# latentnetworks/vimure

Hardware: AMD Instinct MI355X
Metric: CAVI iterations/sec (L=4 N=2000 M=200 K=2 synthetic, mutuality on) (higher is better)
Workload: dtype f64

## Files before the change

### vimure_amd/build.py

```python
import os
import subprocess
from concurrent.futures import ThreadPoolExecutor

HERE = os.path.dirname(os.path.abspath(__file__))
ROOT = os.path.dirname(HERE)
CSRC = os.path.join(HERE, "csrc")
OBJ = os.path.join(CSRC, "_obj")
LIB = os.environ.get("VMR_LIB_OUT", os.path.join(HERE, "libvimure_hip.so"))
HIPCC = os.environ.get("HIPCC", "/opt/rocm/bin/hipcc")
HOST_SRC = os.path.join(CSRC, "host_init.c")
HOST_LIB = os.path.join(HERE, "libvimure_host.so")
HEADERS = [os.path.join(CSRC, "vmr_internal.h"), os.path.join(CSRC, "sweep_sl.h"), os.path.join(CSRC, "sweep_gen.h"),
           os.path.join(CSRC, "sample_draw.h"), os.path.join(CSRC, "report_draw.h"), os.path.join(CSRC, "ppc_layer.h"), os.path.join(CSRC, "rho_row.h"),
           os.path.join(CSRC, "report_lik.h"), os.path.join(CSRC, "read_side.h"), os.path.join(CSRC, "sampled_side.h"),
           os.path.join(ROOT, "include", "vimure_hip.h")]
KS = (2, 3, 4, 5, 6, 7, 8)
FLAGS = ["-O3", "--offload-arch=gfx950", "-fPIC", "-std=c++17", "-I" + os.path.join(ROOT, "include"), "-I" + CSRC]


def units(dev=False):
    extra = ["-DVMR_DEV"] if dev else []
    u = [("vimure_hip", os.path.join(CSRC, "vimure_hip.hip"), extra),
         ("sorted_lists", os.path.join(CSRC, "sorted_lists.hip"), extra),
         ("sweep_gen", os.path.join(CSRC, "sweep_gen.hip"), extra),
         ("generate", os.path.join(CSRC, "generate.hip"), extra),
         ("draw_prior", os.path.join(CSRC, "draw_prior.hip"), extra),
         ("ppc", os.path.join(CSRC, "ppc.hip"), extra),
         ("netstats", os.path.join(CSRC, "netstats.hip"), extra),
         ("triads", os.path.join(CSRC, "triads.hip"), extra),
         ("mixing", os.path.join(CSRC, "mixing.hip"), extra),
         ("ppc_rep", os.path.join(CSRC, "ppc_rep.hip"), extra),
         ("edge_table", os.path.join(CSRC, "edge_table.hip"), extra),
         ("score_truth", os.path.join(CSRC, "score_truth.hip"), extra),
         ("reporter_table", os.path.join(CSRC, "reporter_table.hip"), extra),
         ("heldout", os.path.join(CSRC, "heldout.hip"), extra),
         ("report_scores", os.path.join(CSRC, "report_scores.hip"), extra),
         ("influence", os.path.join(CSRC, "influence.hip"), extra)]
    dev_ks = tuple(int(k) for k in os.environ.get("VMR_DEV_KS", "2").split(","))
    for k in (dev_ks if dev else KS):
        u.append((f"sweep_sl_k{k}", os.path.join(CSRC, "sweep_sl.hip"), extra + [f"-DVMR_K={k}"]))
    return u


def _stale(obj, src):
    if not os.path.exists(obj):
        return True
    t = os.path.getmtime(obj)
    return any(os.path.getmtime(d) > t for d in [src] + HEADERS)


def needs_build() -> bool:
    dev = bool(os.environ.get("VMR_DEV"))
    tag = os.path.join(OBJ, "dev" if dev else "full")
    if not os.path.exists(LIB):
        return True
    t = os.path.getmtime(LIB)
    return any(os.path.getmtime(d) > t for d in [u[1] for u in units(dev)] + HEADERS) or not os.path.exists(tag)


def build(force: bool = False, verbose: bool = False) -> str:
    tagged = bool(os.environ.get("VMR_TAG"))
    if not force and not tagged and not needs_build():
        return LIB
    dev = bool(os.environ.get("VMR_DEV"))
    odir = os.path.join(OBJ, os.environ.get("VMR_TAG") or ("dev" if dev else "full"))
    more = os.environ.get("VMR_CXXFLAGS", "").split()
    os.makedirs(odir, exist_ok=True)
# ... 33 lines not shown
```

### vimure_amd/csrc/sorted_lists.hip

```cpp
#include "sweep_sl.h"

__global__ __launch_bounds__(256) void k_sl_keys(const unsigned* __restrict__ cnt, unsigned* __restrict__ keys, unsigned* __restrict__ vals, size_t T) {
  for (size_t t = (size_t)blockIdx.x * 256 + threadIdx.x; t < T; t += (size_t)gridDim.x * 256) { keys[t] = cnt[t]; vals[t] = (unsigned)t; }
}
__global__ __launch_bounds__(256) void k_sl_level_keys(unsigned* __restrict__ keys, const unsigned* __restrict__ rpl, const unsigned* __restrict__ E,
                                                       size_t T, unsigned rows0, int nb) {
  for (size_t t = (size_t)blockIdx.x * 256 + threadIdx.x; t < T; t += (size_t)gridDim.x * 256) {
    const unsigned r0 = rpl[t], n = rpl[t + 1] - r0;
    unsigned n1 = 0;
    for (unsigned r = 0; r < n; ++r) n1 += SL_YM(E[(size_t)r0 + r]) >= rows0 ? 1u : 0u;
    keys[t] = (n << nb) | n1;
  }
}
__global__ __launch_bounds__(256) void k_sl_steps(const unsigned* __restrict__ keys_sorted, const unsigned* __restrict__ vals_sorted,
                                                  unsigned* __restrict__ sz, unsigned* __restrict__ perm, size_t T, size_t NS, int nb) {
  for (size_t q = (size_t)blockIdx.x * 256 + threadIdx.x; q < NS * 64; q += (size_t)gridDim.x * 256) {
    perm[q] = q < T ? vals_sorted[q] : 0xffffffffu;
    if ((q & 63) == 0) sz[q >> 6] = 64u * (keys_sorted[q] >> nb);
  }
  if (blockIdx.x == 0 && threadIdx.x == 0) sz[NS] = 0u;
}
__global__ __launch_bounds__(256) void k_sl_place(const unsigned* __restrict__ perm, const unsigned* __restrict__ rpl ,
                                                  const unsigned* __restrict__ rsl, const unsigned* __restrict__ Ein,
                                                  unsigned* __restrict__ Eout, const unsigned* __restrict__ Ein2, unsigned* __restrict__ Eout2,
                                                  unsigned* __restrict__ syl, size_t T, size_t NS, int Mp) {
  const int lane = threadIdx.x & 63;
  for (size_t s = (size_t)blockIdx.x * 4 + (threadIdx.x >> 6); s < NS; s += (size_t)gridDim.x * 4) {
    const unsigned t = perm[s * 64 + lane];
    const bool ok = t != 0xffffffffu;
    const unsigned r0 = ok ? rpl[t] : 0u, n = ok ? rpl[t + 1] - r0 : 0u;
    const unsigned ea = rsl[s], R = (rsl[s + 1] - ea) >> 6;
    unsigned rot = 0;
    if (n > 1) { unsigned hsh = t * 0x9E3779B1u; hsh ^= hsh >> 15; hsh *= 0x85EBCA77u; hsh ^= hsh >> 13; rot = hsh % n; }
    unsigned ymx = 0;
    for (unsigned r = 0; r < R; ++r) {
      unsigned q = r + rot;
      if (q >= n) q -= n;
      const unsigned e = n > r ? Ein[(size_t)r0 + q] : 0u;
      Eout[(size_t)ea + r * 64 + lane] = e;
      if (Ein2) Eout2[(size_t)ea + r * 64 + lane] = n > r ? Ein2[(size_t)r0 + q] : 0u;
      ymx = max(ymx, (Ein2 ? e : SL_YM(e)) / (unsigned)Mp);
    }
#pragma unroll
    for (int o2 = 32; o2 > 0; o2 >>= 1) ymx = max(ymx, (unsigned)__shfl_xor((int)ymx, o2, 64));
    if (lane == 0) syl[s] = ymx;
  }
}

template <class V>
__global__ __launch_bounds__(256) void k_sl_gather(const unsigned* __restrict__ perm, const V* __restrict__ in, V* __restrict__ out,
                                                   size_t T, size_t NS, int L) {
  for (size_t q = (size_t)blockIdx.x * 256 + threadIdx.x; q < (size_t)L * T; q += (size_t)gridDim.x * 256) {
    const size_t l = q / T, pos = q - l * T;
    out[q] = in[l * T + perm[l * NS * 64 + pos]];
  }
}
__global__ __launch_bounds__(256) void k_sl_rows(const unsigned* __restrict__ perm, const double* __restrict__ in, double* __restrict__ out,
                                                 size_t T, size_t NS, int L, int K, int to_pos) {
  const size_t n = (size_t)L * T * K;
  for (size_t q = (size_t)blockIdx.x * 256 + threadIdx.x; q < n; q += (size_t)gridDim.x * 256) {
    const size_t row = q / K, k = q - row * K, l = row / T, pos = row - l * T;
    const size_t t = perm[l * NS * 64 + pos];
    if (to_pos) out[q] = in[(l * T + t) * K + k]; else out[(l * T + t) * K + k] = in[q];
  }
}

int sl_permute_u8(vmr_ctx* h, const uint8_t* in, uint8_t* out) {
  const Geo& g = h->g;
  const size_t T = (size_t)g.N * g.N, NS = (T + 63) / 64;
  hipLaunchKernelGGL(k_sl_gather<uint8_t>, dim3((unsigned)std::min<size_t>(8192, (g.L * T + 255) / 256)), dim3(256), 0, h->stream, h->perm, in, out, T, NS, g.L);
  CK(hipGetLastError());
  return VMR_OK;
}
int sl_permute_u32(vmr_ctx* h, const unsigned* in, unsigned* out) {
  const Geo& g = h->g;
  const size_t T = (size_t)g.N * g.N, NS = (T + 63) / 64;
  hipLaunchKernelGGL(k_sl_gather<unsigned>, dim3((unsigned)std::min<size_t>(8192, (g.L * T + 255) / 256)), dim3(256), 0, h->stream, h->perm, in, out, T, NS, g.L);
  CK(hipGetLastError());
  return VMR_OK;
}
int sl_permute_rows(vmr_ctx* h, const double* in, double* out, bool to_pos) {
  const Geo& g = h->g;
  const size_t T = (size_t)g.N * g.N, NS = (T + 63) / 64, n = (size_t)g.L * T * g.K;
  hipLaunchKernelGGL(k_sl_rows, dim3((unsigned)std::min<size_t>(16384, (n + 255) / 256)), dim3(256), 0, h->stream, h->perm, in, out, T, NS, g.L, g.K, to_pos ? 1 : 0);
  HIPCHK(h, hipGetLastError());
  return VMR_OK;
}

int sl_place_entries(vmr_ctx* h, unsigned* rp, const std::vector<unsigned long long>& nl, unsigned* etmp_all, unsigned* etmp2_all, const SlFill* fill) {
  Geo& g = h->g;
  const int L = g.L;
  const size_t T = (size_t)g.N * g.N, n = T + 1, NS = (T + 63) / 64;
  unsigned *keys = nullptr, *keys2 = nullptr, *vals = nullptr, *vals2 = nullptr, *bsum = nullptr, *etmp = nullptr, *etmp2 = nullptr;
  void* tmp = nullptr;
  const bool wide = g.wide != 0;
  auto cleanup = [&]() { void* p[] = {keys, keys2, vals, vals2, bsum, etmp, etmp2, tmp}; for (void* q : p) if (q) (void)hipFree(q); };
#define CKS(call) do { hipError_t e_ = (call); if (e_ != hipSuccess) { g_create_err = std::string(#call) + ": " + hipGetErrorString(e_); (void)hipGetLastError(); cleanup(); return VMR_EHIP; } } while (0)
  if (T >= 0x7fffffffull) return fail(nullptr, VMR_EINVAL, "more than 2^31 ties in one layer");
  CKS(hipMalloc(&keys, T * 4)); CKS(hipMalloc(&keys2, T * 4)); CKS(hipMalloc(&vals, T * 4)); CKS(hipMalloc(&vals2, T * 4));
  CKS(hipMalloc(&bsum, (std::max(n, NS + 1) + 2047) / 2048 * 4));
  CKS(hipMalloc(&h->rs, (size_t)L * (NS + 1) * 4));
  CKS(hipMalloc(&h->perm, (size_t)L * NS * 64 * 4));
  CKS(hipMalloc(&h->sy, (size_t)L * NS * 4));
  size_t tb = 0;
  int bits = 1;
  while (bits < 32 && (1ull << bits) <= (unsigned long long)g.M) ++bits;
  const bool level_keys_ok = !wide && g.mut && 2 * bits <= 30 && !h->opt.no_level_sort;
  CKS(hipcub::DeviceRadixSort::SortPairsDescending(nullptr, tb, keys, keys2, vals, vals2, (int)T, 0, level_keys_ok ? 2 * bits : bits, h->stream));
  CKS(hipMalloc(&tmp, tb ? tb : 8));
  const unsigned tgrid = (unsigned)std::min<size_t>(8192, (T + 255) / 256), sgrid = (unsigned)std::min<size_t>(8192, (NS + 3) / 4);
  if (!etmp_all) {
    unsigned long long nlmax = 0;
    for (int l = 0; l < L; ++l) nlmax = std::max(nlmax, nl[l]);
    CKS(hipMalloc(&etmp, ((size_t)nlmax + 64) * 4));
    if (wide) CKS(hipMalloc(&etmp2, ((size_t)nlmax + 64) * 4));
  }
  unsigned long long off1 = 0;
  for (int l = 0; l < L; ++l) {
    unsigned* rpl = rp + (size_t)l * n;
    unsigned* rsl = h->rs + (size_t)l * (NS + 1);
    const bool by_level = level_keys_ok && (double)nl[l] > (double)SL_PF * (double)T;
    const int nb = by_level ? bits : 0;
    int rc;
    hipLaunchKernelGGL(k_sl_keys, dim3(tgrid), dim3(256), 0, h->stream, rpl, keys, vals, T);
    if (by_level) {
      if ((rc = scan_u32(h, rpl, bsum, n))) { cleanup(); return rc; }
      if (!etmp_all) (*fill)(l, rpl, etmp, etmp2);
      hipLaunchKernelGGL(k_sl_level_keys, dim3(tgrid), dim3(256), 0, h->stream, keys, rpl, etmp_all ? etmp_all + off1 : etmp, T, (unsigned)g.Mp, nb);
    }
    CKS(hipcub::DeviceRadixSort::SortPairsDescending(tmp, tb, keys, keys2, vals, vals2, (int)T, 0, bits + nb, h->stream));
    hipLaunchKernelGGL(k_sl_steps, dim3((unsigned)std::min<size_t>(8192, (NS * 64 + 255) / 256)), dim3(256), 0, h->stream, keys2, vals2, rsl,
                       h->perm + (size_t)l * NS * 64, T, NS, nb);
    CKS(hipGetLastError());
    if ((rc = scan_u32(h, rsl, bsum, NS + 1)) || (!by_level && (rc = scan_u32(h, rpl, bsum, n)))) { cleanup(); return rc; }
    off1 += nl[l];
  }
  CKS(hipStreamSynchronize(h->stream));
  std::vector<unsigned> slots(L);
  for (int l = 0; l < L; ++l) CKS(hipMemcpy(&slots[l], h->rs + (size_t)l * (NS + 1) + NS, 4, hipMemcpyDeviceToHost));
  std::vector<unsigned long long> eb(L);
  h->n_slots = 0;
  for (int l = 0; l < L; ++l) {
    eb[l] = h->n_slots; h->n_slots += slots[l];
    if ((double)slots[l] < (double)nl[l]) { cleanup(); return fail(nullptr, VMR_EINVAL, "more than 2^32 report slots in one layer"); }
  }
  CKS(hipMalloc(&h->ebase, (size_t)L * 8));
  CKS(hipMemcpy(h->ebase, eb.data(), (size_t)L * 8, hipMemcpyHostToDevice));
  CKS(hipMalloc(&h->E, ((size_t)h->n_slots + SL_SLACK) * 4));
  CKS(hipMemsetAsync(h->E + h->n_slots, 0, (size_t)SL_SLACK * 4, h->stream));
  if (wide) {
    CKS(hipMalloc(&h->EX, ((size_t)h->n_slots + SL_SLACK) * 4));
    CKS(hipMemsetAsync(h->EX + h->n_slots, 0, (size_t)SL_SLACK * 4, h->stream));
  }
  unsigned long long off = 0;
  for (int l = 0; l < L; ++l) {
    unsigned* src = etmp_all ? etmp_all + off : etmp;
    unsigned* src2 = wide ? (etmp_all ? etmp2_all + off : etmp2) : nullptr;
    if (!etmp_all) (*fill)(l, rp + (size_t)l * n, etmp, etmp2);
    hipLaunchKernelGGL(k_sl_place, dim3(sgrid), dim3(256), 0, h->stream, h->perm + (size_t)l * NS * 64, rp + (size_t)l * n,
                       h->rs + (size_t)l * (NS + 1), src, h->E + eb[l], src2, wide ? h->EX + eb[l] : nullptr, h->sy + (size_t)l * NS, T, NS, g.Mp);
    off += nl[l];
  }
  CKS(hipGetLastError());
  CKS(hipStreamSynchronize(h->stream));
#undef CKS
  cleanup();
  return VMR_OK;
}

#define SL_DECL(K_) __attribute__((weak)) int vmr_sl_launch_k##K_(vmr_ctx* h, int mode, const SlShape& sh, SlArgs& a);
SL_DECL(2) SL_DECL(3) SL_DECL(4) SL_DECL(5) SL_DECL(6) SL_DECL(7) SL_DECL(8)
#define SL_DECLB(K_) __attribute__((weak)) int vmr_sl_launch_batch_k##K_(vmr_ctx* h, hipStream_t st, int mode, int allfull, const SlUnit* units, const int* blk_unit, int nblocks, int tpb, size_t smem);
SL_DECLB(2) SL_DECLB(3) SL_DECLB(4) SL_DECLB(5) SL_DECLB(6) SL_DECLB(7) SL_DECLB(8)
sl_launch_batch_fn vmr_sl_batch_launcher(int K) {
  switch (K) {
    case 2: return vmr_sl_launch_batch_k2; case 3: return vmr_sl_launch_batch_k3; case 4: return vmr_sl_launch_batch_k4; case 5: return vmr_sl_launch_batch_k5;
    case 6: return vmr_sl_launch_batch_k6; case 7: return vmr_sl_launch_batch_k7; case 8: return vmr_sl_launch_batch_k8;
    default: return nullptr;
  }
}
sl_launch_fn vmr_sl_launcher(int K) {
  switch (K) {
    case 2: return vmr_sl_launch_k2; case 3: return vmr_sl_launch_k3; case 4: return vmr_sl_launch_k4; case 5: return vmr_sl_launch_k5;
    case 6: return vmr_sl_launch_k6; case 7: return vmr_sl_launch_k7; case 8: return vmr_sl_launch_k8;
    default: return nullptr;
  }
}
```

### vimure_amd/csrc/sweep_sl.h

```cpp
#ifndef VMR_SWEEP_SL_H
#define VMR_SWEEP_SL_H

#include "vmr_internal.h"
#include <functional>

#define SL_YM(e) ((e) & 0xfffffu)
#define SL_INR(e) (((e) >> 20) & 1u)
#define SL_X(e) ((e) >> 21)
#define SL_XMAX 2047u
#define SL_YM_ROWS (1u << 20)
#define SL_PF 8
#ifndef SL_PFW
#define SL_PFW 8
#endif
constexpr int sl_pf(int K) { return K <= 2 ? SL_PF : SL_PFW; }
#define SL_SLACK (64 * 64)

struct SlArgs {
  const unsigned* E; const unsigned* rs; const unsigned long long* ebase; const unsigned* perm;
  const unsigned* sy;
  const uint8_t* cls;
  const unsigned* Qt;
  const uint64_t* Rb; const unsigned* rq; const unsigned short* Rm; const unsigned long long* rbase;
  const unsigned* rm2;
// ... 5 lines not shown
  int sum_a;
  double* nu_acc; double* elbo_dev; int commit_nu;
  int nu_stale;
  unsigned long long* det;
  int lp0;
  int farl;
  double* h0s;
  const unsigned* x0p;
  int lv0r;
  const unsigned* Ez;
  int elbo_cur;
  const double* lpd; const double* lpb;
#ifdef SL_DEBUG
  unsigned long long* dbg_t;
#endif
};

struct SlShape { int tpb, yt, hc; size_t smem; };
struct SlUnit { SlArgs a; Geo g; int blk0, nblk; };

#ifndef SL_LIGHT_UPD_K
#define SL_LIGHT_UPD_K 2
#endif
constexpr bool sl_light(int K, bool elbo, bool allfull, bool update) { return !elbo && allfull && (K <= SL_LIGHT_UPD_K || (!update && K <= 4)); }
#ifndef SL_ELBO3_K
#define SL_ELBO3_K 2
#endif
#ifndef SL_ELBO3
#define SL_ELBO3 1
#endif
constexpr int sl_tpb_max(int K, bool elbo, bool allfull, bool update = true) {
  return elbo ? ((SL_ELBO3 && K <= SL_ELBO3_K) ? 768 : (K <= 4 ? 512 : 256)) : (sl_light(K, elbo, allfull, update) ? 1024 : (K <= 3 ? 768 : (K <= 7 ? 512 : 256)));
}
constexpr int sl_tpb_max_b(int K, bool elbo, bool allfull) { return elbo ? sl_tpb_max(K, true, allfull) : (K <= 2 ? 768 : (K <= 7 ? 512 : 256)); }
constexpr int sl_wpe_b(int K, bool elbo, bool allfull) { return elbo ? ((SL_ELBO3 && K <= SL_ELBO3_K) ? 3 : (K <= 4 ? 2 : 1)) : (K <= 2 ? 3 : (K <= 7 ? 2 : 1)); }
constexpr int sl_wpe(int K, bool elbo, bool allfull, bool update = true) {
  return elbo ? ((SL_ELBO3 && K <= SL_ELBO3_K) ? 3 : (K <= 4 ? 2 : 1)) : (sl_light(K, elbo, allfull, update) ? 4 : (K <= 3 ? 3 : (K <= 7 ? 2 : 1)));
}

static inline size_t sl_smem(const Geo& g, int yt, int hc, bool update, bool elbo, bool hist) {
  const size_t lb = (size_t)g.Mp * g.K * 8;
  return (update ? (size_t)yt * lb : 0) + (hist ? (size_t)hc * lb : 0) + (size_t)g.Mp * 8 * (update ? 2 : 1) +
         (size_t)g.W * 8 + 128 + (g.ml ? lb + (size_t)g.Mp * 8 : 0) + (size_t)(64 + (elbo ? 256 : 0)) * 8 + 16;
}

typedef int (*sl_launch_fn)(vmr_ctx* h, int mode, const SlShape& sh, SlArgs& a);
sl_launch_fn vmr_sl_launcher(int K);
typedef int (*sl_launch_batch_fn)(vmr_ctx* h, hipStream_t st, int mode, int allfull, const SlUnit* units, const int* blk_unit, int nblocks,
                                  int tpb, size_t smem);
sl_launch_batch_fn vmr_sl_batch_launcher(int K);

typedef std::function<void(int l, const unsigned* rpl, unsigned* etmp, unsigned* etmp2)> SlFill;
int sl_place_entries(vmr_ctx* h, unsigned* rp, const std::vector<unsigned long long>& nl, unsigned* etmp_all, unsigned* etmp2_all, const SlFill* fill);
int sl_permute_u8(vmr_ctx* h, const uint8_t* in, uint8_t* out);
int sl_permute_u32(vmr_ctx* h, const unsigned* in, unsigned* out);
int sl_permute_rows(vmr_ctx* h, const double* in, double* out, bool to_pos);

#endif
```

### vimure_amd/csrc/vimure_hip.hip

```cpp
#include "vmr_internal.h"
#include "sweep_sl.h"
#include "sweep_gen.h"
#include "sample_draw.h"

thread_local std::string g_create_err;



template <int SH>
__device__ __forceinline__ unsigned nz_flags16(uint4 v) {
  const unsigned M = 0x7f7f7f7fu;
  unsigned t0 = ((v.x & M) + M) | v.x, t1 = ((v.y & M) + M) | v.y;
  unsigned t2 = ((v.z & M) + M) | v.z, t3 = ((v.w & M) + M) | v.w;
  unsigned f = (t0 >> (7 - SH)) & (0x01010101u << SH);
  f |= (t1 >> (6 - SH)) & (0x02020202u << SH);
  f |= (t2 >> (5 - SH)) & (0x04040404u << SH);
  f |= (t3 >> (4 - SH)) & (0x08080808u << SH);
  return f;
}
__device__ __forceinline__ void flag_pos(int bit, int& chunk, int& byte) {
  const int lo = bit & 31;
  chunk = ((bit >> 5) << 1) | ((lo >> 2) & 1);
  byte = ((lo & 3) << 2) | (lo >> 3);
}
// ... 2105 lines not shown
  g.b = b; g.lb = (b == 8) ? 3 : (b == 4) ? 2 : (b == 2) ? 1 : 0;
  g.nb = (g.N + b - 1) / b;
  g.nt = 2 * b * b;
  g.S = TPB / g.nt; if (g.S > 64) g.S = 64;
  g.lS = 0; while ((1 << g.lS) < g.S) ++g.lS;
  g.P = (long long)g.nb * (g.nb + 1) / 2;
  g.Gl = 0;
  g.Y = 1;
  g.hc = 0;
  g.two_pass = 0;
  g.farl = 0;
  g.fuse_full = 0;
  long long T = (long long)g.N * g.N;
  long long gm = (long long)ncu * 8 / g.L; if (gm < 1) gm = 1;
  long long maxgm = (T + 255) / 256; if (gm > maxgm) gm = maxgm; if (gm < 1) gm = 1;
  g.Gm = (int)gm;
  int need = (g.nt * g.nchunk + TPB - 1) / TPB;
  g.pf = need <= 4 ? 4 : need <= 8 ? 8 : 12;
  return VMR_OK;
}

extern "C" {

const char* vmr_version(void) { return VMR_VERSION; }

const char* vmr_last_error(vmr_handle h) { return h ? h->err.c_str() : g_create_err.c_str(); }

}


static void read_opts(VmrOpts& o) {
  memset(&o, 0, sizeof o);
  auto set = [](const char* n) { return getenv(n) != nullptr; };
  auto num = [](const char* n, int dflt) { const char* e = getenv(n); return e ? atoi(e) : dflt; };
  if (const char* f = getenv("VMR_FORMAT")) o.format = !strcmp(f, "dense") ? 1 : !strcmp(f, "sparse") ? 2 : 0;
  o.deterministic = num("VMR_DETERMINISTIC", 0) != 0;
  o.graph = num("VMR_GRAPH", 0) != 0;
  o.debug = num("VMR_DEBUG", 0);
  o.levels = num("VMR_LEVELS", 64);
  o.two_pass = num("VMR_TWO_PASS", 0);
  o.farl = num("VMR_FARL", 0);
  o.yt = set("VMR_YT") ? std::max(0, num("VMR_YT", 0)) : -1;
  o.hc = set("VMR_HC") ? std::max(0, num("VMR_HC", 0)) : -1;
  o.tpb = num("VMR_TPB", 0);
  o.st_tpb = num("VMR_ST_TPB", 0);
  o.no_level0 = set("VMR_NO_LEVEL0");
  o.no_x0 = set("VMR_NO_X0");
  o.no_lv0r = set("VMR_NO_LV0R");
  o.no_level_sort = set("VMR_NO_LEVEL_SORT");
  o.no_rlists = set("VMR_NO_RLISTS");
  o.no_rm2 = set("VMR_NO_RM2");
  o.no_lp0 = set("VMR_NO_LP0");
  o.no_lpd = set("VMR_NO_LPD");
  o.always_store_rho = set("VMR_ALWAYS_STORE_RHO");
  o.debug_lazy_rho = set("VMR_DEBUG_LAZY_RHO");
  o.gen_hsum = num("VMR_GEN_HSUM", 0);
  o.gen_no_lds_h = set("VMR_GEN_NO_LDS_H");
  o.gen_dbg = num("VMR_GEN_DBG", 0);
  o.netstats_chunk = std::max(0, num("VMR_NETSTATS_CHUNK", 0));
  o.batch_fg = set("VMR_BATCH_FG") ? std::max(1, std::min(FG_G, num("VMR_BATCH_FG", 0))) : 0;
  if (const char* t = getenv("VMR_DEBUG_TIMES")) snprintf(o.debug_times, sizeof o.debug_times, "%s", t);
}

static int create_ctx(vmr_ctx** out, hipDeviceProp_t* prop, int device, int L, int N, int M, int K, int mutuality, double eps, bool lists_only = false) {
  if (L < 1 || N < 1 || M < 1) return fail(nullptr, VMR_EINVAL, "L, N, M must be positive");
  if (K < 2 || K > KGEN_MAX) return fail(nullptr, VMR_EINVAL, "K must be in [2, 256]");
  int ndev = 0;
  CK(hipGetDeviceCount(&ndev));
  if (device < 0 || device >= ndev) return fail(nullptr, VMR_EINVAL, "no such HIP device");
  CK(hipSetDevice(device));
  CK(hipGetDeviceProperties(prop, device));
  vmr_ctx* h = new vmr_ctx();
  *out = h;
  h->device = device;
  Geo& g = h->g;
  g.L = L; g.N = N; g.M = M; g.K = K; g.mut = mutuality ? 1 : 0; g.eps = eps;
  g.gen = K > KMAX ? 1 : 0; g.wide = 0;
  read_opts(h->opt);
  g.dbg = h->opt.debug;
  g.det = h->opt.deterministic ? 1 : 0; g.det_sh = 0; g.det_shr = 0; g.det_sha = 0;
  std::string err;
  if (choose_geo(g, prop->multiProcessorCount, err, lists_only) != VMR_OK) return fail(nullptr, VMR_EINVAL, err.c_str());
  memset(h->prof_ms, 0, sizeof h->prof_ms); memset(h->prof_n, 0, sizeof h->prof_n);
  CK(hipStreamCreateWithFlags(&h->stream, hipStreamNonBlocking));
  CK(hipStreamCreateWithFlags(&h->stream2, hipStreamNonBlocking));
  CK(hipEventCreateWithFlags(&h->ev_fork, hipEventDisableTiming));
  CK(hipEventCreateWithFlags(&h->ev_join, hipEventDisableTiming));
  h->ncu = prop->multiProcessorCount;
  h->use_graphs = h->opt.graph;
  const size_t rows = (size_t)L * N * N;
  CK(hipMalloc(&h->cov, rows));
  CK(hipMalloc(&h->rcls, rows));
  CK(hipMalloc(&h->sumx, 8));
  CK(hipMemsetAsync(h->sumx, 0, 8, h->stream));
  CK(hipMalloc(&h->xmax, 4));
  CK(hipMemsetAsync(h->xmax, 0, 4, h->stream));
  CK(hipMalloc(&h->npartial, 16));
  CK(hipMemsetAsync(h->npartial, 0, 16, h->stream));
  return VMR_OK;
}

static int create_state(vmr_ctx* h, unsigned* xm_out) {
  Geo& g = h->g;
  const size_t rows = (size_t)g.L * g.N * g.N;
  CK(hipMalloc(&h->rho, (rows + 64) * g.K * 8));
  CK(hipMalloc(&h->logpr, (rows + 64) * g.K * 8));
// ... 70 lines not shown
    for (int l = 0; l < L; ++l)
      hipLaunchKernelGGL(k_rm_fill, dim3(rgrid), dim3(256), 0, h->stream, h->Rb + (size_t)l * T * g.W,
                         h->rcls + (size_t)l * T, h->rq + (size_t)l * n, h->Rm + rb_[l], T, g.W);
    CK(hipGetLastError());
    CK(hipStreamSynchronize(h->stream));
  } else {
    CK(hipFree(h->rq));
    h->rq = nullptr;
    h->n_rm = 0;
  }
  CK(hipFree(bsum));
  return VMR_OK;
}

__global__ __launch_bounds__(256) void k_level_hist(const unsigned* __restrict__ E, unsigned long long n, int Mp, unsigned long long* __restrict__ hist) {
  __shared__ unsigned long long sh[65];
  for (int i = threadIdx.x; i < 65; i += 256) sh[i] = 0;
  __syncthreads();
  for (unsigned long long i = (unsigned long long)blockIdx.x * 256 + threadIdx.x; i < n; i += (unsigned long long)gridDim.x * 256) {
    const unsigned e = E[i];
    if (e == 0u) continue;
    const unsigned y = SL_YM(e) / (unsigned)Mp;
    atomicAdd(&sh[y < 64u ? y : 64u], 1ull);
  }
  __syncthreads();
  for (int i = threadIdx.x; i < 65; i += 256) if (sh[i]) atomicAdd(&hist[i], sh[i]);
}

static int build_far_lists(vmr_ctx* h) {
  const Geo& g = h->g;
  const size_t T = (size_t)g.N * g.N, NS = (T + 63) / 64;
  unsigned long long* cnt = nullptr;
  unsigned long long* hd = nullptr;
  struct Tmp { unsigned long long*& a; unsigned long long*& b; ~Tmp() { if (a) (void)hipFree(a); if (b) (void)hipFree(b); } } tmp_guard{cnt, hd};
  CK(hipMalloc(&cnt, 8));
  std::vector<unsigned long long> hist(65, 0);
  CK(hipMalloc(&hd, 65 * 8));
  CK(hipMemsetAsync(hd, 0, 65 * 8, h->stream));
  hipLaunchKernelGGL(k_level_hist, dim3(1024), dim3(256), 0, h->stream, h->E, h->n_slots, g.Mp, hd);
  CK(hipGetLastError());
  CK(hipMemcpyAsync(hist.data(), hd, 65 * 8, hipMemcpyDeviceToHost, h->stream));
  CK(hipStreamSynchronize(h->stream));
  unsigned long long far = 0;
  for (int y = std::min(g.hc, 64); y < 65; ++y) far += hist[y];
  CK(hipMalloc(&h->far_pos, (size_t)(far + 64) * 4));
  CK(hipMalloc(&h->far_ent, (size_t)(far + 64) * 4));
  h->far_off.assign(g.L + 1, 0ull);
  std::vector<unsigned long long> eb(g.L);
  CK(hipMemcpy(eb.data(), h->ebase, (size_t)g.L * 8, hipMemcpyDeviceToHost));
  for (int l = 0; l < g.L; ++l) {
    hipLaunchKernelGGL(k_far_first, dim3((unsigned)std::min<size_t>(8192, (NS + 3) / 4)), dim3(256), 0, h->stream, h->E + eb[l], h->rs + (size_t)l * (NS + 1),
                       h->sy + (size_t)l * NS, NS, (unsigned)g.hc * (unsigned)g.Mp, (unsigned*)nullptr);
    CK(hipGetLastError());
    CK(hipMemsetAsync(cnt, 0, 8, h->stream));
    hipLaunchKernelGGL(k_far_collect, dim3((unsigned)std::min<size_t>(8192, (NS + 3) / 4)), dim3(256), 0, h->stream, h->E + eb[l], h->rs + (size_t)l * (NS + 1), NS,
                       (unsigned)g.hc * (unsigned)g.Mp, h->far_pos + h->far_off[l], h->far_ent + h->far_off[l], cnt);
    CK(hipGetLastError());
    unsigned long long n = 0;
    CK(hipMemcpyAsync(&n, cnt, 8, hipMemcpyDeviceToHost, h->stream));
    CK(hipStreamSynchronize(h->stream));
    h->far_off[l + 1] = h->far_off[l] + n;
    if (h->far_off[l + 1] > far) return fail(nullptr, VMR_EHIP, "far lists: more reports than counted");
  }
  CK(hipMalloc(&h->far_base, (size_t)(g.L + 1) * 8));
  CK(hipMemcpy(h->far_base, h->far_off.data(), (size_t)(g.L + 1) * 8, hipMemcpyHostToDevice));
  return VMR_OK;
}

__global__ __launch_bounds__(256) void k_rm2(const unsigned* __restrict__ perm, const unsigned* __restrict__ rq, const unsigned short* __restrict__ Rm,
                                             const unsigned long long* __restrict__ rbase, unsigned* __restrict__ out, size_t T, size_t NS, int L) {
  const size_t n = (size_t)L * NS * 64;
  for (size_t q = (size_t)blockIdx.x * 256 + threadIdx.x; q < n; q += (size_t)gridDim.x * 256) {
    const size_t l = q / (NS * 64);
    const unsigned tie = perm[q];
    unsigned w = 0xffffffffu;
    if (tie != 0xffffffffu) {
      const unsigned q0 = rq[l * (T + 1) + tie], q1 = rq[l * (T + 1) + tie + 1];
      const unsigned short* r = Rm + rbase[l];
      const unsigned m0 = q1 > q0 ? r[q0] : 0xffffu, m1 = q1 > q0 + 1 ? r[q0 + 1] : 0xffffu;
      w = m0 | (m1 << 16);
    }
    out[q] = w;
  }
}

static int sl_finish(vmr_ctx* h) {
  const Geo& g = h->g;
  const size_t rows = (size_t)g.L * g.N * g.N;
  int rc = VMR_OK;
  if (!h->all_full) {
    CK(hipMalloc(&h->cls_p, rows + 64));
    CK(hipMemsetAsync(h->cls_p + rows, 0, 64, h->stream));
    if ((rc = sl_permute_u8(h, h->rcls, h->cls_p))) return rc;
  }
  if (g.mut && h->Qt) {
    CK(hipMalloc(&h->Qt_p, (rows + 64) * 4));
    CK(hipMemsetAsync(h->Qt_p + rows, 0, 64 * 4, h->stream));
    if ((rc = sl_permute_u32(h, h->Qt, h->Qt_p))) return rc;
    CK(hipStreamSynchronize(h->stream));
    CK(hipFree(h->Qt)); h->Qt = nullptr;
  }
  return VMR_OK;
}

static int det_scales(vmr_ctx* h, int xbits, int shr_max) {
  Geo& g = h->g;
// ... 81 lines not shown
        int bw = 0, bt = 256;
        for (int tpb : {1024, 768, 512, 256}) { const int w = waves(tpb, upd ? lv : 0, hist ? lv : 0, upd, hist); if (w > bw) { bw = w; bt = tpb; } }
        if (bw >= min_waves) { lv_out = lv; tpb_out = bt; return true; }
      }
      return false;
    };
    int lv1 = 0, t1 = 256, lvr = 0, tr = 256, lvh = 0, th = 256;
    bool want_farl = false;
    bool one = best(true, true, 16, lv1, t1);
    if (one && lv1 < want && g.N > 1024) {
      std::vector<unsigned long long> hist(65, 0);
      unsigned long long* hd = nullptr;
      CK(hipMalloc(&hd, 65 * 8));
      CK(hipMemsetAsync(hd, 0, 65 * 8, h->stream));
      hipLaunchKernelGGL(k_level_hist, dim3(1024), dim3(256), 0, h->stream, h->E, h->n_slots, g.Mp, hd);
      CK(hipGetLastError());
      CK(hipMemcpyAsync(hist.data(), hd, 65 * 8, hipMemcpyDeviceToHost, h->stream));
      CK(hipStreamSynchronize(h->stream));
      CK(hipFree(hd));
      unsigned long long tot = 0, far = 0;
      for (int y = 0; y < 65; ++y) { tot += hist[y]; if (y >= lv1) far += hist[y]; }
      if ((double)far > (double)tot / 1024.0) {
        if (g.mut && !g.det && o.farl && (double)far <= 0.125 * (double)tot) want_farl = true;
        else one = false;
      }
    }
    one = one && !o.two_pass;
    if (one) { g.yt = g.hc = lv1; h->sp_tpb = h->st_tpb = t1; g.farl = want_farl ? 1 : 0; }
    else {
      g.two_pass = 1;
      if (!best(true, false, 16, lvr, tr) && !best(true, false, 4, lvr, tr)) { lvr = 0; tr = 256; }
      if (!best(false, true, 16, lvh, th) && !best(false, true, 4, lvh, th)) { lvh = 0; th = 256; }
      g.yt = lvr; g.hc = lvh; h->sp_tpb = tr; h->st_tpb = th;
    }
    {
      const long long NS = ((long long)g.N * g.N + 63) / 64;
      for (int* t : {&h->sp_tpb, &h->st_tpb})
        while (*t > 64 && NS * L < (long long)h->ncu * (*t / 64)) *t = std::max(64, (*t / 2) & ~63);
    }
    g.yt = std::max(0, std::min(g.Y, o.yt >= 0 ? o.yt : g.yt));
    g.hc = std::max(0, std::min(g.Y, o.hc >= 0 ? o.hc : g.hc));
    if (o.tpb >= 64 && o.tpb <= 1024 && o.tpb % 64 == 0) h->sp_tpb = o.tpb;
    if (o.st_tpb >= 64 && o.st_tpb <= 1024 && o.st_tpb % 64 == 0) h->st_tpb = o.st_tpb;
    for (int v = 0; v < 4; ++v) need = std::max(need, sl_shape(h, v != 3, v == 1 || v == 2, v == 0 || v == 1 || v == 3).smem);
    if (g.two_pass && g.mut && !g.det && g.Y > 1 && !o.no_level0) {
      const size_t T_ = (size_t)g.N * g.N, NS_ = (T_ + 63) / 64;
      std::vector<unsigned long long> eb(L);
      CK(hipMemcpy(eb.data(), h->ebase, (size_t)L * 8, hipMemcpyDeviceToHost));
      if (!o.no_x0) CK(hipMalloc(&h->x0p, (size_t)L * NS_ * 64 * 4));
      for (int l = 0; l < L; ++l)
        hipLaunchKernelGGL(k_far_first, dim3((unsigned)std::min<size_t>(8192, (NS_ + 3) / 4)), dim3(256), 0, h->stream, h->E + eb[l], h->rs + (size_t)l * (NS_ + 1),
                           h->sy + (size_t)l * NS_, NS_, (unsigned)g.Mp, h->x0p ? h->x0p + (size_t)l * NS_ * 64 : nullptr);
      CK(hipGetLastError());
      if (h->x0p) {
        unsigned long long* ss = nullptr;
        CK(hipMalloc(&ss, 8));
        CK(hipMemsetAsync(ss, 0, 8, h->stream));
        for (int l = 0; l < L; ++l)
          hipLaunchKernelGGL(k_stat_slots, dim3(256), dim3(256), 0, h->stream, h->rs + (size_t)l * (NS_ + 1), h->sy + (size_t)l * NS_, NS_, ss);
        hipError_t es = hipMemcpyAsync(&h->stat_slots, ss, 8, hipMemcpyDeviceToHost, h->stream);
        if (es == hipSuccess) es = hipStreamSynchronize(h->stream);
        (void)hipFree(ss);
        CK(es);
      }
      const size_t n0 = (size_t)L * NSLOT * K + L;
      CK(hipMalloc(&h->h0s, n0 * 8));
      CK(hipMemsetAsync(h->h0s, 0, n0 * 8, h->stream));
    }
    if (g.farl) {
      bool same = g.hc >= 1 && g.hc < g.Y;
      for (int v : {0, 3}) same = same && sl_shape(h, v != 3, false, true).hc == g.hc;
      h->elbo_split = sl_shape(h, true, true, true).hc != g.hc || sl_shape(h, true, true, true).yt != g.yt;
      if (!same) g.farl = 0;
      else { int rcf = build_far_lists(h); if (rcf) return rcf; }
    }
  } else {
    if (shmem_rho(g, true, false) > 80000) {
      g.two_pass = 1;
      while (g.hc > 0 && shmem_hist(g) > 160000) --g.hc;
    }
    need = std::max(shmem_rho(g, true, true), shmem_hist(g));
  }
  if (need > (size_t)prop.sharedMemPerBlock && need > 160 * 1024) {
    char msg[256];
    snprintf(msg, sizeof msg, "M = %d reporters with K = %d%s needs %zu bytes of LDS per workgroup (limit %d): "
             "reduce M or K", g.M, K, g.mut ? " and mutuality" : "", need, 160 * 1024);
    return fail(nullptr, VMR_EINVAL, msg);
  }
  CK(hipMalloc(&h->Hg, (size_t)L * NH * g.Y * g.Mp * K * 8));
  CK(hipMemsetAsync(h->Hg, 0, (size_t)L * NH * g.Y * g.Mp * K * 8, h->stream));
  CK(hipMalloc(&h->elbo_dev, 8 * 8));
  CK(hipMemsetAsync(h->elbo_dev, 0, 8 * 8, h->stream));
  CK(hipMalloc(&h->nu_acc, (size_t)(3 + L) * 8));
  CK(hipMemsetAsync(h->nu_acc, 0, (size_t)(3 + L) * 8, h->stream));
  CK(hipMalloc(&h->fin_g, ((size_t)L * (2 * KMAX + 2) + (size_t)L * FG_G * 2 * KMAX) * 8));
  CK(hipMemsetAsync(h->fin_g, 0, ((size_t)L * (2 * KMAX + 2) + (size_t)L * FG_G * 2 * KMAX) * 8, h->stream));
  if (g.det) {
    if (!h->sparse) return fail(nullptr, VMR_EINVAL, "VMR_DETERMINISTIC=1 needs the report lists (a sparse tensor with M <= 8192, counts <= 2047)");
    int rc = det_scales(h, 11, 45);
    if (rc) return rc;
    const unsigned long long T_ = (unsigned long long)g.N * g.N;
    int tbits = 1;
    while (tbits < 62 && (T_ >> tbits) != 0ull) ++tbits;
    g.det_sha = std::min(42, 62 - tbits);
    const size_t nd = (size_t)L * g.Y * g.Mp * K + (size_t)L * g.W * 64 * K + (size_t)L * K + 5;
    CK(hipMalloc(&h->det_buf, nd * 8));
// ... 1324 lines not shown
```

### vimure_amd/csrc/vmr_internal.h

```cpp
#ifndef VMR_INTERNAL_H
#define VMR_INTERNAL_H
#include <hip/hip_runtime.h>
#include <hipcub/hipcub.hpp>
#include <stdint.h>
#include <stdio.h>
#include <string.h>
#include <math.h>
#include <stdlib.h>
#include <string>
#include <vector>
#include <utility>
#include <algorithm>
#include <chrono>
#include <type_traits>

#include "vimure_hip.h"

#define VMR_VERSION "vimure_hip 0.1 (gfx950)"
#define TPB 256
#ifndef VMR_LB_COUNTS
#define VMR_LB_COUNTS 4
#endif
#ifndef VMR_LB_RHO
#define VMR_LB_RHO 3
#endif
#ifndef VMR_NR_STEPS
#define VMR_NR_STEPS 1
#endif
#define KMAX 8
#define KGEN_MAX 256

struct Geo {
  int L, N, M, K, mut;
  int Mp;
  int nchunk;
  int stride;
  int W;
  int b, lb;
  int nb;
  int nt;
  int S, lS;
  long long P;
  int Gl;
  int Gm;
  int Y;
  int hc;
  int yt;
  int fuse_full;
  int ml;
  int two_pass;
  int pf;
  int dbg;
  double eps;
  int det;
  int det_sh;
  int det_shr;
  int gen;
  int farl;
  int wide;
  int det_sha;
};
#define DET_SH2 30
__device__ __forceinline__ unsigned long long det_fx(double v, int sh) { return (unsigned long long)__double2ll_rn(ldexp(v, sh)); }
__device__ __forceinline__ double det_back(unsigned long long u, int sh) { return ldexp((double)(long long)u, -sh); }

#define NSLOT 8

struct VmrOpts {
  int format;
  bool deterministic, graph;
  int debug, levels;
  int two_pass, farl;
  int yt, hc;
  int tpb, st_tpb;
  bool no_level0, no_x0, no_lv0r, no_level_sort, no_rlists, no_rm2, no_lp0, no_lpd;
  bool always_store_rho, debug_lazy_rho;
  int gen_hsum;
  bool gen_no_lds_h;
  int gen_dbg;
  int batch_fg;
  int netstats_chunk;
  char debug_times[256];
};

struct vmr_ctx {
  Geo g;
  VmrOpts opt;
  int device;
  hipStream_t stream;
  hipStream_t stream2 = nullptr;
  hipEvent_t ev_fork = nullptr, ev_join = nullptr;
  std::string err;
  uint8_t* X = nullptr;
  uint64_t* Rb = nullptr;
  uint8_t* cov = nullptr;
  void* drw = nullptr;
  size_t drw_cap = 0;
  uint8_t* rcls = nullptr;
  int sparse = 0;
  unsigned* E = nullptr;
  unsigned* EX = nullptr;
  double* gen_s1 = nullptr;
  unsigned* rs = nullptr;
  double* Cg = nullptr;
  int sp_tpb = 256;
  int st_tpb = 256;
  unsigned* Qt = nullptr;
  unsigned long long* ebase = nullptr;
  unsigned long long nnz = 0;
  unsigned long long n_slots = 0;
  int all_full = 0;
  unsigned* perm = nullptr;
  unsigned* sy = nullptr;
  unsigned* far_pos = nullptr;
  unsigned* far_ent = nullptr;
  unsigned long long* far_base = nullptr;
  std::vector<unsigned long long> far_off;
  double* h0s = nullptr;
  unsigned long long stat_slots = 0;
  unsigned* x0p = nullptr;
  bool elbo_split = false;
  uint8_t* cls_p = nullptr;
  unsigned* Qt_p = nullptr;
  double* nat = nullptr;
  unsigned* rq = nullptr;
  unsigned short* Rm = nullptr;
  unsigned long long* rbase = nullptr;
  unsigned long long n_rm = 0;
// ... 306 lines not shown
```

Baseline: 6080.

## Rebalance sorted-list slot rounds to reduce LDS bank and read-group conflicts

Adds a setup-time kernel that permutes, within windows of eight rounds, the entries each lane handles in a sorted-list step. It greedily assigns and then pairwise-swaps entries to even out per-round counts of row reads and LDS bank accesses across lane groups. A window is written back only when the new arrangement is no worse by that cost measure. This targets bank and row-read contention in the sweep kernels and adds a one-time preprocessing pass; it relies on reordering within the lead/tail segments being semantically neutral.

```diff
diff --git a/vimure_amd/build.py b/vimure_amd/build.py
--- a/vimure_amd/build.py
+++ b/vimure_amd/build.py
@@ -12,7 +12,7 @@
 HOST_LIB = os.path.join(HERE, "libvimure_host.so")
 HEADERS = [os.path.join(CSRC, "vmr_internal.h"), os.path.join(CSRC, "sweep_sl.h"), os.path.join(CSRC, "sweep_gen.h"),
            os.path.join(CSRC, "sample_draw.h"), os.path.join(CSRC, "report_draw.h"), os.path.join(CSRC, "ppc_layer.h"), os.path.join(CSRC, "rho_row.h"),
-           os.path.join(CSRC, "report_lik.h"), os.path.join(CSRC, "read_side.h"), os.path.join(CSRC, "sampled_side.h"),
+           os.path.join(CSRC, "report_lik.h"), os.path.join(CSRC, "read_side.h"), os.path.join(CSRC, "sampled_side.h"), os.path.join(CSRC, "sl_balance.h"),
            os.path.join(ROOT, "include", "vimure_hip.h")]
 KS = (2, 3, 4, 5, 6, 7, 8)
 FLAGS = ["-O3", "--offload-arch=gfx950", "-fPIC", "-std=c++17", "-I" + os.path.join(ROOT, "include"), "-I" + CSRC]
diff --git a/vimure_amd/csrc/sl_balance.h b/vimure_amd/csrc/sl_balance.h
--- /dev/null
+++ b/vimure_amd/csrc/sl_balance.h
@@ -0,0 +1,144 @@
+#ifndef VMR_SL_BALANCE_H
+#define VMR_SL_BALANCE_H
+
+#if defined(__HIPCC__)
+#define SLB_HD __host__ __device__
+#else
+#define SLB_HD
+#endif
+
+#define SLB_WIN 8
+#define SLB_CHAINS 4
+#define SLB_ROW(e) ((e) & 0xfffffu)
+
+struct SlbScratch {
+  unsigned char cr[SLB_WIN][4][16];
+  unsigned char ca[SLB_WIN][4][16];
+  unsigned in[SLB_WIN * 64];
+};
+
+SLB_HD inline int slb_read_group(int lane) {
+  const int q = lane & 31;
+  return ((lane >> 5) << 1) | (int)((0xf00f0ff0u >> q) & 1u);
+}
+
+SLB_HD inline int slb_group_lane(int g, int i) {
+  const int q = (g & 1) ? (i < 8 ? i + 4 : (i < 12 ? i + 8 : i + 16)) : (i < 4 ? i : (i < 8 ? i + 8 : i + 12));
+  return ((g >> 1) << 5) + q;
+}
+
+SLB_HD inline int slb_chain_lane(int p, int c, int i) {
+  const int half = (c >> 1) << 5, upper = (c & 1) << 4;
+  const int q = p == 0 ? (i < 4 ? i : i + 8) : i + 4;
+  return half + upper + q;
+}
+
+SLB_HD inline bool slb_opens_row(const unsigned* w, int lane) {
+  const unsigned e = w[lane];
+  const int g = slb_read_group(lane);
+  bool dup = false;
+  for (int i = 0; i < 16; ++i) {
+    const int j = slb_group_lane(g, i);
+    const unsigned o = w[j];
+    dup = dup || (j < lane && o != 0u && SLB_ROW(o) == SLB_ROW(e));
+  }
+  return e != 0u && !dup;
+}
+
+inline void slb_round_cost(const unsigned* w, unsigned* rd, unsigned* ad) {
+  unsigned nrow[4][16] = {}, nlane[4][16] = {};
+  for (int lane = 0; lane < 64; ++lane) {
+    if (w[lane] == 0u) continue;
+    const unsigned s = SLB_ROW(w[lane]) & 15u;
+    ++nlane[lane >> 4][s];
+    if (slb_opens_row(w, lane)) ++nrow[slb_read_group(lane)][s];
+  }
+  for (int g = 0; g < 4; ++g) {
+    unsigned mr = 0u, ma = 0u;
+    for (int s = 0; s < 16; ++s) { mr = nrow[g][s] > mr ? nrow[g][s] : mr; ma = nlane[g][s] > ma ? nlane[g][s] : ma; }
+    *rd += mr; *ad += ma;
+  }
+}
+
+SLB_HD inline void slb_place_lane(unsigned* w, int nr, int lane, unsigned lead, unsigned n, SlbScratch* sc) {
+  const int gr = slb_read_group(lane), ga = lane >> 4;
+  const int nl = (int)n < nr ? (int)n : nr, ld = (int)lead < nl ? (int)lead : nl;
+  for (int seg = 0; seg < 2; ++seg) {
+    const int lo = seg ? ld : 0, hi = seg ? nl : ld;
+    unsigned used = 0u;
+    for (int i = lo; i < hi; ++i) {
+      const unsigned e = sc->in[i * 64 + lane], s = SLB_ROW(e) & 15u;
+      int best = -1; unsigned bc = 0u;
+      for (int r = lo; r < hi; ++r) {
+        const unsigned c = (unsigned)sc->cr[r][gr][s] + (unsigned)sc->ca[r][ga][s];
+        if (!((used >> r) & 1u) && (best < 0 || c < bc)) { best = r; bc = c; }
+      }
+      used |= 1u << best;
+      w[best * 64 + lane] = e;
+      ++sc->cr[best][gr][s]; ++sc->ca[best][ga][s];
+    }
+  }
+}
+
+SLB_HD inline void slb_refine_lane(unsigned* w, int nr, int lane, unsigned lead, unsigned n, SlbScratch* sc) {
+  const int gr = slb_read_group(lane), ga = lane >> 4;
+  const int nl = (int)n < nr ? (int)n : nr, ld = (int)lead < nl ? (int)lead : nl;
+  for (int seg = 0; seg < 2; ++seg) {
+    const int lo = seg ? ld : 0, hi = seg ? nl : ld;
+    for (int a = lo; a < hi; ++a)
+      for (int b = a + 1; b < hi; ++b) {
+        const unsigned ea = w[a * 64 + lane], eb = w[b * 64 + lane], sa = SLB_ROW(ea) & 15u, sb = SLB_ROW(eb) & 15u;
+        if (sa == sb) continue;
+        const int now = (int)sc->cr[a][gr][sa] + (int)sc->ca[a][ga][sa] + (int)sc->cr[b][gr][sb] + (int)sc->ca[b][ga][sb] - 4;
+        const int then = (int)sc->cr[a][gr][sb] + (int)sc->ca[a][ga][sb] + (int)sc->cr[b][gr][sa] + (int)sc->ca[b][ga][sa];
+        if (then < now) {
+          --sc->cr[a][gr][sa]; --sc->ca[a][ga][sa]; --sc->cr[b][gr][sb]; --sc->ca[b][ga][sb];
+          ++sc->cr[a][gr][sb]; ++sc->ca[a][ga][sb]; ++sc->cr[b][gr][sa]; ++sc->ca[b][ga][sa];
+          w[a * 64 + lane] = eb; w[b * 64 + lane] = ea;
+        }
+      }
+  }
+}
+
+SLB_HD inline void slb_chain_phase(unsigned* w, int nr, const unsigned* lead, const unsigned* n, SlbScratch* sc, int c, int p, bool refine) {
+  for (int i = 0; i < 8; ++i) {
+    const int lane = slb_chain_lane(p, c, i);
+    if (refine) slb_refine_lane(w, nr, lane, lead[lane], n[lane], sc);
+    else slb_place_lane(w, nr, lane, lead[lane], n[lane], sc);
+  }
+}
+
+inline void slb_balance_window(unsigned* w, int nr, const unsigned* lead, const unsigned* n, SlbScratch* sc) {
+  if (nr < 2) return;
+  for (int i = 0; i < nr * 64; ++i) sc->in[i] = w[i];
+  for (int r = 0; r < nr; ++r)
+    for (int g = 0; g < 4; ++g)
+      for (int s = 0; s < 16; ++s) { sc->cr[r][g][s] = 0; sc->ca[r][g][s] = 0; }
+  for (int pass = 0; pass < 2; ++pass)
+    for (int p = 0; p < 2; ++p)
+      for (int c = 0; c < SLB_CHAINS; ++c) slb_chain_phase(w, nr, lead, n, sc, c, p, pass == 1);
+  unsigned r0 = 0u, a0 = 0u, r1 = 0u, a1 = 0u;
+  for (int r = 0; r < nr; ++r) { slb_round_cost(sc->in + r * 64, &r0, &a0); slb_round_cost(w + r * 64, &r1, &a1); }
+  if (r1 > r0 || a1 > a0)
+    for (int i = 0; i < nr * 64; ++i) w[i] = sc->in[i];
+}
+
+SLB_HD inline unsigned slb_clip(unsigned v, unsigned r0) { return v > r0 ? v - r0 : 0u; }
+
+SLB_HD inline unsigned slb_count(const unsigned* col, unsigned R) {
+  unsigned n = 0u;
+  for (unsigned r = 0; r < R; ++r) if (col[(unsigned long long)r * 64] != 0u) n = r + 1;
+  return n;
+}
+
+inline void slb_balance_step(unsigned* e, unsigned R, const unsigned* lead, SlbScratch* sc) {
+  unsigned n[64], lw[64], nw[64];
+  for (int lane = 0; lane < 64; ++lane) n[lane] = slb_count(e + lane, R);
+  for (unsigned r0 = 0; r0 < R; r0 += SLB_WIN) {
+    const unsigned nr = R - r0 < SLB_WIN ? R - r0 : SLB_WIN;
+    for (int lane = 0; lane < 64; ++lane) { lw[lane] = slb_clip(lead[lane] < n[lane] ? lead[lane] : n[lane], r0); nw[lane] = slb_clip(n[lane], r0); }
+    slb_balance_window(e + (unsigned long long)r0 * 64, (int)nr, lw, nw, sc);
+  }
+}
+
+#endif
diff --git a/vimure_amd/csrc/sorted_lists.hip b/vimure_amd/csrc/sorted_lists.hip
--- a/vimure_amd/csrc/sorted_lists.hip
+++ b/vimure_amd/csrc/sorted_lists.hip
@@ -1,4 +1,5 @@
 #include "sweep_sl.h"
+#include "sl_balance.h"
 
 __global__ __launch_bounds__(256) void k_sl_keys(const unsigned* __restrict__ cnt, unsigned* __restrict__ keys, unsigned* __restrict__ vals, size_t T) {
   for (size_t t = (size_t)blockIdx.x * 256 + threadIdx.x; t < T; t += (size_t)gridDim.x * 256) { keys[t] = cnt[t]; vals[t] = (unsigned)t; }
@@ -46,6 +47,67 @@
     if (lane == 0) syl[s] = ymx;
   }
 }
+__global__ __launch_bounds__(64) __attribute__((amdgpu_waves_per_eu(7))) void k_sl_balance(unsigned* __restrict__ E, const unsigned* __restrict__ rsl, size_t NS, unsigned rows_near) {
+  __shared__ unsigned win[SLB_WIN * 64];
+  __shared__ unsigned lead[64], cnt[64];
+  __shared__ SlbScratch sc;
+  __shared__ unsigned tot[16];
+  static_assert(sizeof sc.cr + sizeof sc.ca == 2 * 8 * 16 * sizeof(unsigned) && offsetof(SlbScratch, ca) == sizeof sc.cr, "hist aliases cr | ca");
+  unsigned (*hist)[8][16] = reinterpret_cast<unsigned (*)[8][16]>(&sc.cr[0][0][0]);
+  const int lane = threadIdx.x;
+  for (size_t s = blockIdx.x; s < NS; s += gridDim.x) {
+    const unsigned ea = rsl[s], R = (rsl[s + 1] - ea) >> 6;
+    if (R < 2) break;
+    unsigned* col = E + (size_t)ea + lane;
+    unsigned n = 0, ld = 0;
+    for (unsigned r = 0; r < R; ++r) {
+      const unsigned e = col[(size_t)r * 64];
+      if (e != 0u) n = r + 1;
+      if (r == ld && e != 0u && SL_YM(e) >= rows_near) ++ld;
+    }
+    for (unsigned r0 = 0; r0 < R; r0 += SLB_WIN) {
+      const unsigned nr = min((unsigned)SLB_WIN, R - r0);
+      if (nr < 2) break;
+      for (unsigned r = 0; r < nr; ++r) { const unsigned e = col[(size_t)(r0 + r) * 64]; win[r * 64 + lane] = e; sc.in[r * 64 + lane] = e; }
+      lead[lane] = slb_clip(min(ld, n), r0);
+      cnt[lane] = slb_clip(n, r0);
+      for (int i = lane; i < SLB_WIN * 4 * 16; i += 64) { (&sc.cr[0][0][0])[i] = 0; (&sc.ca[0][0][0])[i] = 0; }
+      __syncthreads();
+      for (int pass = 0; pass < 2; ++pass)
+        for (int p = 0; p < 2; ++p) {
+          if (lane < SLB_CHAINS) slb_chain_phase(win, (int)nr, lead, cnt, &sc, lane, p, pass == 1);
+          __syncthreads();
+        }
+      unsigned acc = 0;
+      for (unsigned r = 0; r < nr; ++r) {
+        for (int i = lane; i < 2 * 8 * 16; i += 64) (&hist[0][0][0])[i] = 0u;
+        __syncthreads();
+        for (int a = 0; a < 2; ++a) {
+          const unsigned* w = (a ? win : sc.in) + r * 64;
+          const unsigned e = w[lane];
+          if (e != 0u) {
+            atomicAdd(&hist[a][4 + (lane >> 4)][SLB_ROW(e) & 15u], 1u);
+            if (slb_opens_row(w, lane)) atomicAdd(&hist[a][slb_read_group(lane)][SLB_ROW(e) & 15u], 1u);
+          }
+        }
+        __syncthreads();
+        if (lane < 16) {
+          unsigned m = 0;
+          for (int s = 0; s < 16; ++s) m = max(m, hist[lane >> 3][lane & 7][s]);
+          acc += m;
+        }
+        __syncthreads();
+      }
+      if (lane < 16) tot[lane] = acc;
+      __syncthreads();
+      const unsigned rd0 = tot[0] + tot[1] + tot[2] + tot[3], ad0 = tot[4] + tot[5] + tot[6] + tot[7];
+      const unsigned rd1 = tot[8] + tot[9] + tot[10] + tot[11], ad1 = tot[12] + tot[13] + tot[14] + tot[15];
+      if (rd1 <= rd0 && ad1 <= ad0)
+        for (unsigned r = 0; r < nr; ++r) col[(size_t)(r0 + r) * 64] = win[r * 64 + lane];
+      __syncthreads();
+    }
+  }
+}
 
 template <class V>
 __global__ __launch_bounds__(256) void k_sl_gather(const unsigned* __restrict__ perm, const V* __restrict__ in, V* __restrict__ out,
@@ -84,6 +146,15 @@
   const size_t T = (size_t)g.N * g.N, NS = (T + 63) / 64, n = (size_t)g.L * T * g.K;
   hipLaunchKernelGGL(k_sl_rows, dim3((unsigned)std::min<size_t>(16384, (n + 255) / 256)), dim3(256), 0, h->stream, h->perm, in, out, T, NS, g.L, g.K, to_pos ? 1 : 0);
   HIPCHK(h, hipGetLastError());
+  return VMR_OK;
+}
+
+int sl_balance_layer(vmr_ctx* h, int l, unsigned long long eb, unsigned rows_near) {
+  const Geo& g = h->g;
+  if (g.wide || h->opt.no_balance) return VMR_OK;
+  const size_t T = (size_t)g.N * g.N, NS = (T + 63) / 64;
+  hipLaunchKernelGGL(k_sl_balance, dim3((unsigned)std::min<size_t>(1u << 20, NS)), dim3(64), 0, h->stream, h->E + eb, h->rs + (size_t)l * (NS + 1), NS, rows_near);
+  CK(hipGetLastError());
   return VMR_OK;
 }
 
@@ -162,6 +233,7 @@
     off += nl[l];
   }
   CKS(hipGetLastError());
+  for (int l = 0; l < L; ++l) { const int rc = sl_balance_layer(h, l, eb[l], 0xffffffffu); if (rc) { cleanup(); return rc; } }
   CKS(hipStreamSynchronize(h->stream));
 #undef CKS
   cleanup();
diff --git a/vimure_amd/csrc/sweep_sl.h b/vimure_amd/csrc/sweep_sl.h
--- a/vimure_amd/csrc/sweep_sl.h
+++ b/vimure_amd/csrc/sweep_sl.h
@@ -81,6 +81,7 @@
 
 typedef std::function<void(int l, const unsigned* rpl, unsigned* etmp, unsigned* etmp2)> SlFill;
 int sl_place_entries(vmr_ctx* h, unsigned* rp, const std::vector<unsigned long long>& nl, unsigned* etmp_all, unsigned* etmp2_all, const SlFill* fill);
+int sl_balance_layer(vmr_ctx* h, int l, unsigned long long eb, unsigned rows_near);
 int sl_permute_u8(vmr_ctx* h, const uint8_t* in, uint8_t* out);
 int sl_permute_u32(vmr_ctx* h, const unsigned* in, unsigned* out);
 int sl_permute_rows(vmr_ctx* h, const double* in, double* out, bool to_pos);
diff --git a/vimure_amd/csrc/vimure_hip.hip b/vimure_amd/csrc/vimure_hip.hip
--- a/vimure_amd/csrc/vimure_hip.hip
+++ b/vimure_amd/csrc/vimure_hip.hip
@@ -2181,6 +2181,7 @@
   o.no_rm2 = set("VMR_NO_RM2");
   o.no_lp0 = set("VMR_NO_LP0");
   o.no_lpd = set("VMR_NO_LPD");
+  o.no_balance = set("VMR_NO_BALANCE");
   o.always_store_rho = set("VMR_ALWAYS_STORE_RHO");
   o.debug_lazy_rho = set("VMR_DEBUG_LAZY_RHO");
   o.gen_hsum = num("VMR_GEN_HSUM", 0);
@@ -2357,6 +2358,7 @@
     hipLaunchKernelGGL(k_far_first, dim3((unsigned)std::min<size_t>(8192, (NS + 3) / 4)), dim3(256), 0, h->stream, h->E + eb[l], h->rs + (size_t)l * (NS + 1),
                        h->sy + (size_t)l * NS, NS, (unsigned)g.hc * (unsigned)g.Mp, (unsigned*)nullptr);
     CK(hipGetLastError());
+    { const int rcb = sl_balance_layer(h, l, eb[l], (unsigned)g.hc * (unsigned)g.Mp); if (rcb) return rcb; }
     CK(hipMemsetAsync(cnt, 0, 8, h->stream));
     hipLaunchKernelGGL(k_far_collect, dim3((unsigned)std::min<size_t>(8192, (NS + 3) / 4)), dim3(256), 0, h->stream, h->E + eb[l], h->rs + (size_t)l * (NS + 1), NS,
                        (unsigned)g.hc * (unsigned)g.Mp, h->far_pos + h->far_off[l], h->far_ent + h->far_off[l], cnt);
@@ -2544,6 +2546,7 @@
         hipLaunchKernelGGL(k_far_first, dim3((unsigned)std::min<size_t>(8192, (NS_ + 3) / 4)), dim3(256), 0, h->stream, h->E + eb[l], h->rs + (size_t)l * (NS_ + 1),
                            h->sy + (size_t)l * NS_, NS_, (unsigned)g.Mp, h->x0p ? h->x0p + (size_t)l * NS_ * 64 : nullptr);
       CK(hipGetLastError());
+      for (int l = 0; l < L; ++l) { const int rcb = sl_balance_layer(h, l, eb[l], (unsigned)g.Mp); if (rcb) return rcb; }
       if (h->x0p) {
         unsigned long long* ss = nullptr;
         CK(hipMalloc(&ss, 8));
diff --git a/vimure_amd/csrc/vmr_internal.h b/vimure_amd/csrc/vmr_internal.h
--- a/vimure_amd/csrc/vmr_internal.h
+++ b/vimure_amd/csrc/vmr_internal.h
@@ -73,7 +73,7 @@
   int two_pass, farl;
   int yt, hc;
   int tpb, st_tpb;
-  bool no_level0, no_x0, no_lv0r, no_level_sort, no_rlists, no_rm2, no_lp0, no_lpd;
+  bool no_level0, no_x0, no_lv0r, no_level_sort, no_rlists, no_rm2, no_lp0, no_lpd, no_balance;
   bool always_store_rho, debug_lazy_rho;
   int gen_hsum;
   bool gen_no_lds_h;
```

New measurement: 6343 (median of 6 runs). 1.04x the previous value.
